# zhizdev/sparsefusion

Measured on AMD Instinct MI355X. Metric: novel views/sec, distillation steps (2 NGP renders fwd+bwd + VAE enc/dec + 51-eval PLMS + LPIPS), 256^2 / 32x32 latents, 2-view synthetic hydrant, higher is better.
Workload: dtype bf16 MFMA operands / f32 accumulate (UNet); f32 (NGP render)

## Files before the change

### include/sparsefusion_hip.h

```cpp
#ifndef SPARSEFUSION_HIP_H
#define SPARSEFUSION_HIP_H

#include <stdint.h>

#ifdef __cplusplus
extern "C" {
#endif

#define SF_OK 0
#define SF_ERR_INVALID 1
#define SF_ERR_LAUNCH 2

const char* sf_last_error(void);
int sf_abi_version(void);
int sf_operand_is_f16(void);


int sf_grid_encode_forward(const float* inputs, const float* embeddings,
                           const int32_t* offsets, float* outputs,
                           uint32_t B, uint32_t D, uint32_t C, uint32_t L,
                           float S, uint32_t H, float* dy_dx,
                           uint32_t gridtype, int align_corners,
                           const int32_t* h_offsets, void* stream);

// ... 116 lines not shown
                         const uint32_t* faces_per_label, const uint32_t* counts3, uint32_t min_faces, double min_fraction,
                         void* workspace, uint64_t workspace_bytes, uint32_t* counts2, void* stream);
int sf_mesh_filter_emit(const float* verts, const int32_t* faces, uint32_t F, uint32_t V, void* workspace,
                        uint64_t workspace_bytes, float* out_verts, int32_t* out_faces, int32_t* vertex_ids, int32_t* face_ids,
                        void* stream);

int sf_ngp_render_forward(const sf_ngp_field* f, const float* rays_o,
                          const float* rays_d, const float* aabb, uint32_t N,
                          uint32_t T, float min_near, const float* lin,
                          const float* u_coarse, const float* u_fine,
                          uint32_t u_fine_row_stride, float bg_color, float* nears,
                          float* fars, float* z_sorted, float* sigma_s,
                          float* rgb_s, float* image, float* depth,
                          float* weights_sum, float* field_cache, float* workspace,
                          uint64_t workspace_bytes, void* stream);

int sf_ngp_render_backward(const sf_ngp_field* f, const sf_ngp_field_grad* g,
                           const float* rays_o, const float* rays_d,
                           const float* aabb, uint32_t N, uint32_t T,
                           const float* nears, const float* fars,
                           const float* z_sorted, const float* sigma_s,
                           const float* rgb_s, float bg_color,
                           const float* grad_image, const float* grad_weights_sum,
                           uint32_t rays_per_row, const float* field_cache,
                           float* workspace, uint64_t workspace_bytes,
                           void* stream);

uint64_t sf_ngp_render_workspace_bytes(uint32_t N, uint32_t T);
uint64_t sf_ngp_render_forward_workspace_bytes(uint32_t N, uint32_t T);

uint64_t sf_ngp_render_cache_bytes(uint32_t N, uint32_t T);

int sf_ngp_field_mfma(int on);

int sf_ngp_field_bwd_pipe(int on);
void sf_ngp_field_bwd_launches(uint64_t* counts);

int sf_ngp_render_shaded_forward(const sf_ngp_field* f, const float* rays_o, const float* rays_d, const float* aabb,
                                 uint32_t N, uint32_t T, float min_near, const float* lin, const float* u_coarse,
                                 const float* u_fine, uint32_t u_fine_row_stride, float bg_color, const float* light_d,
                                 float ambient_ratio, float epsilon, float* nears, float* fars, float* z_sorted,
                                 float* sigma_s, float* rgb_s, float* normal_s, float* rgb_shaded_s, float* xyz_s,
                                 float* image, float* normal_image, float* orient, float* depth, float* weights_sum,
                                 float* workspace, uint64_t workspace_bytes, void* stream);
uint64_t sf_ngp_render_shaded_workspace_bytes(uint32_t N, uint32_t T);

int sf_ngp_render_shaded_forward_train(const sf_ngp_field* f, const float* rays_o, const float* rays_d, const float* aabb,
                                       uint32_t N, uint32_t T, float min_near, const float* lin, const float* u_coarse,
                                       const float* u_fine, uint32_t u_fine_row_stride, float bg_color, const float* light_d,
                                       float ambient_ratio, float epsilon, float* nears, float* fars, float* z_sorted,
                                       float* sigma_s, float* rgb_s, float* normal_s, float* rgb_shaded_s, float* grad_s,
                                       float* w_s, float* image, float* normal_image, float* orient, float* depth,
                                       float* weights_sum, float* workspace, uint64_t workspace_bytes, void* stream);
int sf_ngp_render_shaded_backward(const sf_ngp_field* f, const sf_ngp_field_grad* g, const float* rays_o, const float* rays_d,
                                  const float* aabb, uint32_t N, uint32_t T, const float* nears, const float* fars,
                                  const float* z_sorted, const float* sigma_s, const float* rgb_s, const float* normal_s,
                                  const float* rgb_shaded_s, const float* grad_s, const float* w_s, const float* light_d,
                                  float ambient_ratio, float epsilon, float bg_color, const float* grad_image,
                                  const float* grad_weights_sum, const float* grad_orient, uint32_t rays_per_row,
                                  float* workspace, uint64_t workspace_bytes, void* stream);
uint64_t sf_ngp_render_shaded_backward_workspace_bytes(uint32_t N, uint32_t T);
int sf_ngp_render_offset_backward(const sf_ngp_field* f, const sf_ngp_field_grad* g, const float* rays_o, const float* rays_d,
                                  const float* aabb, uint32_t N, uint32_t T, const float* z_sorted, const float* ds_e, uint32_t e,
                                  float epsilon, uint32_t rays_per_row, float* workspace, uint64_t workspace_bytes, void* stream);

int sf_ngp_render_occ_eval(const sf_ngp_field* f, const float* rays_o, const float* rays_d,
// ... 103 lines not shown
```

### sparsefusion_amd/_lib.py

```python
import ctypes as C
import os

import torch

_HERE = os.path.dirname(os.path.abspath(__file__))
_DEFAULT_LIB = "libsparsefusion_hip_f16.so" if os.environ.get("SF_OPERAND", "bf16").lower() in ("f16", "fp16", "half") else "libsparsefusion_hip.so"
LIB_PATH = os.environ.get("SF_HIP_LIB") or os.path.join(_HERE, _DEFAULT_LIB)

_lib = None

c_f32p = C.c_void_p
c_i32p = C.c_void_p
u32 = C.c_uint32
u64 = C.c_uint64


class SfNgpField(C.Structure):
    _fields_ = [("embeddings", C.c_void_p), ("h_offsets", C.c_void_p), ("L", u32), ("S", C.c_float),
                ("H", u32), ("gridtype", u32),
                ("w0", C.c_void_p), ("b0", C.c_void_p), ("w1", C.c_void_p), ("b1", C.c_void_p),
                ("w2", C.c_void_p), ("b2", C.c_void_p), ("bound", C.c_float)]


class SfNgpFieldGrad(C.Structure):
# ... 51 lines not shown
    "sf_upsample2x_backward": (C.c_int, [c_f32p, c_f32p, u32, u32, u32, C.c_void_p]),
    "sf_render_loss_forward": (C.c_int, [c_f32p, c_f32p, c_f32p, c_f32p, u64, u64, C.c_float, c_f32p, C.c_void_p]),
    "sf_render_loss_backward": (C.c_int, [c_f32p, c_f32p, c_f32p, c_f32p, u64, u64, C.c_float, C.c_float, C.c_float, C.c_float,
                                          C.c_float, c_f32p, c_f32p, c_f32p, C.c_void_p]),
    "sf_fusion_loss_forward": (C.c_int, [c_f32p, c_f32p, c_f32p, c_f32p, u32, u64, u64, c_f32p, C.c_void_p]),
    "sf_fusion_loss_backward": (C.c_int, [c_f32p, c_f32p, c_f32p, c_f32p, u32, u64, u64, C.c_float, C.c_float, C.c_float,
                                          c_f32p, c_f32p, c_f32p, C.c_void_p]),
    "sf_ngp_density": (C.c_int, [C.POINTER(SfNgpField), c_f32p, u32, c_f32p, c_f32p, C.c_void_p]),
    "sf_ngp_density_lattice": (C.c_int, [C.POINTER(SfNgpField), c_f32p, c_f32p, c_f32p, u32, u32, u32, c_f32p, C.c_void_p]),
    "sf_ngp_point_attrs": (C.c_int, [C.POINTER(SfNgpField), c_f32p, u32, C.c_float, c_f32p, c_f32p, c_f32p, c_f32p, C.c_void_p]),
    "sf_ngp_texture_bake": (C.c_int, [C.POINTER(SfNgpField), c_f32p, u32, c_i32p, u32, u32, C.c_void_p, c_f32p, c_f32p, c_i32p,
                                      C.c_void_p]),
    "sf_gaussian3d_workspace_bytes": (u64, [u32, u32, u32]),
    "sf_gaussian3d": (C.c_int, [c_f32p, c_f32p, u32, u32, u32, C.c_float, C.c_float, C.c_void_p, C.c_void_p, u64, C.c_void_p]),
    "sf_mc_workspace_bytes": (u64, [u32, u32, u32]),
    "sf_mc_count": (C.c_int, [c_f32p, u32, u32, u32, C.c_float, C.c_void_p, u64, C.c_void_p, C.c_void_p]),
    "sf_mc_emit": (C.c_int, [c_f32p, u32, u32, u32, C.c_float, C.c_void_p, u64, c_f32p, c_i32p, C.c_void_p]),
    "sf_mesh_components_workspace_bytes": (u64, [u32, u32]),
    "sf_mesh_components": (C.c_int, [c_i32p, u32, u32, c_i32p, c_i32p, C.c_void_p, C.c_void_p, C.c_void_p, u64, C.c_void_p]),
    "sf_mesh_filter_workspace_bytes": (u64, [u32, u32]),
    "sf_mesh_filter_count": (C.c_int, [c_i32p, u32, u32, c_i32p, C.c_void_p, C.c_void_p, u32, C.c_double, C.c_void_p, u64,
                                       C.c_void_p, C.c_void_p]),
    "sf_mesh_filter_emit": (C.c_int, [c_f32p, c_i32p, u32, u32, C.c_void_p, u64, c_f32p, c_i32p, c_i32p, c_i32p, C.c_void_p]),
    "sf_ngp_render_forward": (C.c_int, [C.POINTER(SfNgpField), c_f32p, c_f32p, c_f32p, u32, u32, C.c_float,
                                        c_f32p, c_f32p, c_f32p, u32, C.c_float, c_f32p, c_f32p, c_f32p, c_f32p,
                                        c_f32p, c_f32p, c_f32p, c_f32p, c_f32p, c_f32p, u64, C.c_void_p]),
    "sf_ngp_render_backward": (C.c_int, [C.POINTER(SfNgpField), C.POINTER(SfNgpFieldGrad), c_f32p, c_f32p,
                                         c_f32p, u32, u32, c_f32p, c_f32p, c_f32p, c_f32p, c_f32p,
                                         C.c_float, c_f32p, c_f32p, u32, c_f32p, c_f32p, u64, C.c_void_p]),
    "sf_ngp_render_workspace_bytes": (u64, [u32, u32]),
    "sf_ngp_render_forward_workspace_bytes": (u64, [u32, u32]),
    "sf_ngp_render_cache_bytes": (u64, [u32, u32]),
    "sf_ngp_field_mfma": (C.c_int, [C.c_int]),
    "sf_ngp_field_bwd_pipe": (C.c_int, [C.c_int]),
    "sf_ngp_field_bwd_launches": (None, [C.c_void_p]),
    "sf_ngp_render_shaded_forward": (C.c_int, [C.POINTER(SfNgpField), c_f32p, c_f32p, c_f32p, u32, u32, C.c_float, c_f32p, c_f32p,
                                               c_f32p, u32, C.c_float, c_f32p, C.c_float, C.c_float, c_f32p, c_f32p, c_f32p,
                                               c_f32p, c_f32p, c_f32p, c_f32p, c_f32p, c_f32p, c_f32p, c_f32p, c_f32p, c_f32p,
                                               c_f32p, u64, C.c_void_p]),
    "sf_ngp_render_shaded_workspace_bytes": (u64, [u32, u32]),
    "sf_ngp_render_shaded_forward_train": (C.c_int, [C.POINTER(SfNgpField), c_f32p, c_f32p, c_f32p, u32, u32, C.c_float, c_f32p, c_f32p,
                                                     c_f32p, u32, C.c_float, c_f32p, C.c_float, C.c_float, c_f32p, c_f32p, c_f32p,
                                                     c_f32p, c_f32p, c_f32p, c_f32p, c_f32p, c_f32p, c_f32p, c_f32p, c_f32p, c_f32p,
                                                     c_f32p, c_f32p, u64, C.c_void_p]),
    "sf_ngp_render_shaded_backward": (C.c_int, [C.POINTER(SfNgpField), C.POINTER(SfNgpFieldGrad), c_f32p, c_f32p, c_f32p, u32, u32,
                                                c_f32p, c_f32p, c_f32p, c_f32p, c_f32p, c_f32p, c_f32p, c_f32p, c_f32p, c_f32p,
                                                C.c_float, C.c_float, C.c_float, c_f32p, c_f32p, c_f32p, u32, c_f32p, u64, C.c_void_p]),
    "sf_ngp_render_shaded_backward_workspace_bytes": (u64, [u32, u32]),
    "sf_ngp_render_offset_backward": (C.c_int, [C.POINTER(SfNgpField), C.POINTER(SfNgpFieldGrad), c_f32p, c_f32p, c_f32p, u32, u32, c_f32p,
                                                c_f32p, u32, C.c_float, u32, c_f32p, u64, C.c_void_p]),
    "sf_ngp_render_occ_eval": (C.c_int, [C.POINTER(SfNgpField), c_f32p, c_f32p, c_f32p, c_f32p, C.c_void_p, C.c_float, u32, u32, u32,
                                         c_f32p, C.c_float, u32, c_f32p, c_f32p, c_f32p, C.c_void_p]),
    "sf_ngp_render_occ_eval_shaded": (C.c_int, [C.POINTER(SfNgpField), c_f32p, c_f32p, c_f32p, c_f32p, C.c_void_p, C.c_float, u32, u32,
                                                u32, c_f32p, C.c_float, u32, c_f32p, C.c_float, C.c_float, c_f32p, c_f32p, c_f32p,
                                                c_f32p, C.c_void_p, C.c_void_p]),
    "sf_plan_run": (C.c_int, [C.POINTER(SfOp), u32, C.c_void_p]),
    "sf_conv_igemm_t_launches": (u64, []),
    "sf_gca4_launches": (u64, [C.c_int]),
    "sf_plan_profile": (C.c_int, [C.POINTER(SfOp), u32, C.c_void_p, C.c_void_p]),
    "sf_conv_packed_elems": (u64, [u32, u32, u32, u32]),
    "sf_conv_pack_weights": (C.c_int, [C.c_void_p, u32, u32, u32, u32, u32, C.c_void_p]),
    "sf_plms_update": (C.c_int, [c_f32p, c_f32p, c_f32p, C.c_void_p, u64, c_f32p, c_f32p, C.c_void_p]),
    "sf_plms_combine": (C.c_int, [c_f32p, c_f32p, c_f32p, c_f32p, C.c_void_p, u64, c_f32p, c_f32p, C.c_void_p]),
    "sf_plms_step": (C.c_int, [c_f32p, c_f32p, c_f32p, c_f32p, C.c_void_p, c_f32p, c_f32p, c_f32p, C.c_void_p, u64, c_f32p, c_f32p, c_f32p, u64, C.c_void_p]),
}

# ... 55 lines not shown
```

### sparsefusion_amd/csrc/ngp_field_mfma.h

```cpp
#pragma once
#include "sf_dev.h"
#include "ngp_device.h"

#define FM_PTS 32
#define FM_SF 33
#define FM_SH 65
#define FM_WAVE_FLOATS (FM_PTS * FM_SF + FM_PTS * FM_SH)
#define FM_W2 0
#define FM_B2 (FM_W2 + NGP_OUT * NGP_HID)
#define FM_B0 (FM_B2 + 8)
#define FM_B1 (FM_B0 + NGP_HID)
#define FM_W0 (FM_B1 + NGP_HID)
#define FM_HEAD (FM_W0 + NGP_HID * FM_SF)
#define FM_LDS_FLOATS (FM_HEAD + 4 * FM_WAVE_FLOATS)

#ifndef FM_DEPTH
#define FM_DEPTH 1
#endif

#ifdef SF_HOST_EMU
#define FM_SCHED_FENCE() do { } while (0)
#else
#define FM_SCHED_FENCE() __builtin_amdgcn_sched_barrier(0)
#endif

struct FMArgs {
  const float* table; const float* w0; const float* b0; const float* w1; const float* b1; const float* w2; const float* b2;
  float bound;
  NgpLevels lv;
  const float* rays_o; const float* rays_d; const float* aabb; const float* nears; const float* fars;
  const float* lin; const float* u;
  const float* z_in;
  uint32_t P, T;
  float* z_out;
  float* sigma; float* rgb;
  float* feat_out;
};

SF_DEV void fm_level(const NgpLevels& lv, uint32_t hi, int ll, NgpLevels& m) {
  m.scale[0] = hi ? lv.scale[8 + ll] : lv.scale[ll];
  m.resolution[0] = hi ? lv.resolution[8 + ll] : lv.resolution[ll];
  m.offset[0] = hi ? lv.offset[8 + ll] : lv.offset[ll];
  m.hsize[0] = hi ? lv.hsize[8 + ll] : lv.hsize[ll];
  m.gridtype = lv.gridtype;
}

template <int MODE>
SF_KERNEL(256) void k_ngp_field_mfma(FMArgs a) {
  SF_DYN_LDS(lds_raw);
  float* W = reinterpret_cast<float*>(lds_raw);
  const int tid = threadIdx.x, lane = tid & 63, wave = tid >> 6;
  const int li = lane & 15, kq = lane >> 4;
  float bw1[NGP_HID / 4][4];
  {
    float* S1 = W + FM_HEAD;
    for (int i = tid; i < NGP_HID * NGP_FEAT; i += 256) W[FM_W0 + (i >> 5) * FM_SF + (i & 31)] = a.w0[i];
    for (int i = tid; i < NGP_HID * NGP_HID; i += 256) S1[(i >> 6) * FM_SH + (i & 63)] = a.w1[i];
    for (int i = tid; i < NGP_OUT * NGP_HID; i += 256) W[FM_W2 + i] = a.w2[i];
    if (tid < NGP_HID) { W[FM_B0 + tid] = a.b0[tid]; W[FM_B1 + tid] = a.b1[tid]; }
    if (tid < NGP_OUT) W[FM_B2 + tid] = a.b2[tid];
    sf_sync();
#pragma unroll
    for (int nt = 0; nt < 4; ++nt) {
#pragma unroll
      for (int s = 0; s < NGP_HID / 4; ++s) bw1[s][nt] = S1[(nt * 16 + li) * FM_SH + 4 * s + kq];
    }
    sf_sync();
  }
  float* F = W + FM_HEAD + wave * FM_WAVE_FLOATS;
  float* H = F + FM_PTS * FM_SF;
  float box[6];
#pragma unroll
  for (int i = 0; i < 6; ++i) box[i] = a.aabb[i];

  const int pl = lane & 31, half = lane >> 5;
  const uint32_t n_trips = (a.P + FM_PTS - 1) / FM_PTS;
  for (uint32_t trip = blockIdx.x * 4 + wave; trip < n_trips; trip += gridDim.x * 4) {
    const uint32_t p = trip * FM_PTS + pl;
    const bool live = p < a.P;
    float x01[3] = {0.f, 0.f, 0.f}, blob = 0.0f;
    bool inside = false;
    if (live) {
      const uint32_t n = p / a.T;
      float z;
      if (MODE == 0) {
        z = ngp_coarse_z(a.nears[n], a.fars[n], a.lin[p - n * a.T], a.u ? a.u[p] : -1.0f, a.T);
        if (half == 0) a.z_out[p] = z;
      } else {
        z = a.z_in[p];
      }
      const float o[3] = {a.rays_o[n * 3], a.rays_o[n * 3 + 1], a.rays_o[n * 3 + 2]};
      const float d[3] = {a.rays_d[n * 3], a.rays_d[n * 3 + 1], a.rays_d[n * 3 + 2]};
      float x[3];
      ngp_point(o, d, z, box, x);
      inside = ngp_unit(x, a.bound, x01);
      blob = ngp_blob(x);
    }
    const float xe[3] = {inside ? x01[0] : 0.0f, inside ? x01[1] : 0.0f, inside ? x01[2] : 0.0f};
    uint32_t hi = half;
    SF_USE_FROM_HERE(hi);
    f32x2 fv[FM_DEPTH][8];
    float w[FM_DEPTH][8];
    NgpCell c;
    NgpLevels m;
#pragma unroll
    for (int q = 0; q < FM_DEPTH; ++q) {
      fm_level(a.lv, hi, q, m);
      ngp_cell(m, 0, xe, c);
      const float* tab = a.table + (size_t)m.offset[0] * 2;
#pragma unroll
      for (int i = 0; i < 8; ++i) {
        fv[q][i] = *reinterpret_cast<const f32x2*>(tab + (size_t)c.row[i] * 2);
        w[q][i] = c.w[i];
      }
      FM_SCHED_FENCE();
    }
#pragma unroll
    for (int ll = 0; ll < 8; ++ll) {
      const uint32_t l = hi * 8 + ll;
      const int q = ll % FM_DEPTH;
      const float* tab = a.table;
      if (ll + FM_DEPTH < 8) {
        fm_level(a.lv, hi, ll + FM_DEPTH, m);
        ngp_cell(m, 0, xe, c);
        tab = a.table + (size_t)m.offset[0] * 2;
      }
      FM_SCHED_FENCE();
      float r0 = 0.0f, r1 = 0.0f;
#pragma unroll
      for (int i = 0; i < 8; ++i) {
        r0 = fmaf(w[q][i], fv[q][i][0], r0);
        r1 = fmaf(w[q][i], fv[q][i][1], r1);
      }
      if (!(inside && l < a.lv.L)) r0 = r1 = 0.0f;
      F[pl * FM_SF + 2 * l] = r0;
      F[pl * FM_SF + 2 * l + 1] = r1;
      if (ll + FM_DEPTH < 8) {
#pragma unroll
        for (int i = 0; i < 8; ++i) {
          fv[q][i] = *reinterpret_cast<const f32x2*>(tab + (size_t)c.row[i] * 2);
          w[q][i] = c.w[i];
        }
      }
      FM_SCHED_FENCE();
    }
    if (a.feat_out && live) {
      float* dst = a.feat_out + (size_t)p * NGP_FEAT + half * 16;
#pragma unroll
      for (int j = 0; j < 4; ++j) {
        f32x4 v;
#pragma unroll
        for (int e = 0; e < 4; ++e) v[e] = F[pl * FM_SF + half * 16 + 4 * j + e];
        *reinterpret_cast<f32x4*>(dst + 4 * j) = v;
      }
    }
    sf_wave_sync();

#pragma unroll
    for (int mt = 0; mt < 2; ++mt) {
      f32x4 c[4];
#pragma unroll
      for (int nt = 0; nt < 4; ++nt) {
        const float bv = W[FM_B0 + nt * 16 + li];
        c[nt] = f32x4{bv, bv, bv, bv};
      }
#pragma unroll
      for (int s = 0; s < NGP_FEAT / 4; ++s) {
        const float av = F[(mt * 16 + li) * FM_SF + 4 * s + kq];
#pragma unroll
        for (int nt = 0; nt < 4; ++nt) c[nt] = sf_mfma4(av, W[FM_W0 + (nt * 16 + li) * FM_SF + 4 * s + kq], c[nt]);
      }
#pragma unroll
      for (int nt = 0; nt < 4; ++nt)
#pragma unroll
        for (int r = 0; r < 4; ++r) H[(mt * 16 + 4 * kq + r) * FM_SH + nt * 16 + li] = fmaxf(c[nt][r], 0.0f);
    }
    sf_wave_sync();
#pragma unroll
    for (int mt = 0; mt < 2; ++mt) {
      f32x4 c[4];
#pragma unroll
      for (int nt = 0; nt < 4; ++nt) {
        const float bv = W[FM_B1 + nt * 16 + li];
        c[nt] = f32x4{bv, bv, bv, bv};
      }
#pragma unroll
      for (int s = 0; s < NGP_HID / 4; ++s) {
        const float av = H[(mt * 16 + li) * FM_SH + 4 * s + kq];
#pragma unroll
        for (int nt = 0; nt < 4; ++nt) c[nt] = sf_mfma4(av, bw1[s][nt], c[nt]);
      }
      sf_wave_sync();
#pragma unroll
      for (int nt = 0; nt < 4; ++nt)
#pragma unroll
        for (int r = 0; r < 4; ++r) H[(mt * 16 + 4 * kq + r) * FM_SH + nt * 16 + li] = fmaxf(c[nt][r], 0.0f);
    }
    sf_wave_sync();
    {
      float o0 = W[FM_B2 + 2 * half], o1 = W[FM_B2 + 2 * half + 1];
#pragma unroll 8
      for (int k = 0; k < NGP_HID; ++k) {
        const float hk = H[pl * FM_SH + k];
        o0 = fmaf(W[FM_W2 + (2 * half) * NGP_HID + k], hk, o0);
        o1 = fmaf(W[FM_W2 + (2 * half + 1) * NGP_HID + k], hk, o1);
      }
      if (live) {
        if (half == 0) {
          a.sigma[p] = expf(o0 + blob);
          a.rgb[(size_t)p * 3 + 0] = ngp_sigmoid(o1);
        } else {
          a.rgb[(size_t)p * 3 + 1] = ngp_sigmoid(o0);
          a.rgb[(size_t)p * 3 + 2] = ngp_sigmoid(o1);
        }
      }
    }
    sf_wave_sync();
  }
}
```

### sparsefusion_amd/csrc/ngp_render.hip

```cpp

#include "sf_common.h"
#include "ngp_device.h"
#include "ngp_bwd_plan.h"
#include "ngp_field_lds.h"
#include "ngp_bwd_mfma.h"
#include "ngp_bwd_pipe.h"
#include "ngp_field_mfma.h"
#include "ngp_composite_wave.h"
#include "ngp_scatter_bin.h"
#include "ngp_shade.h"
#include "ngp_shade_bwd.h"
#include <stdlib.h>
#include <atomic>
#include <mutex>

struct GridLevels;
int sf_fill_levels(GridLevels* lv, const int32_t* offsets_dev, const int32_t* h_offsets, uint32_t L, float S,
                   uint32_t H, hipStream_t st);

template <int MODE>
__global__ __launch_bounds__(256) void k_ngp_field(
    FieldPtrs f, NgpLevels lv, const float* __restrict__ rays_o, const float* __restrict__ rays_d,
    const float* __restrict__ aabb, const float* __restrict__ nears, const float* __restrict__ fars,
    const float* __restrict__ lin, const float* __restrict__ u, const float* __restrict__ z_in,
// ... 240 lines not shown
  out->gridtype = f->gridtype;
  return SF_OK;
}

static FieldPtrs field_ptrs(const sf_ngp_field* f) { return sf_ngp_field_ptrs(f); }

extern "C" int sf_ngp_density(const sf_ngp_field* f, const float* xyz, uint32_t P, float* sigma, float* albedo,
                              void* stream) {
  hipStream_t st = (hipStream_t)stream;
  NgpLevels lv;
  if (int rc = sf_ngp_make_levels(f, &lv, st)) return rc;
  if (P == 0) return SF_OK;
  k_ngp_field<2><<<sf_grid_cap(sf_div_up(P, 256)), 256, 0, st>>>(field_ptrs(f), lv, nullptr, nullptr, nullptr, nullptr,
                                                                 nullptr, nullptr, nullptr, nullptr, xyz, P, 1, nullptr,
                                                                 sigma, albedo);
  SF_CHECK_LAUNCH("ngp_density");
  return SF_OK;
}

extern "C" uint64_t sf_ngp_render_workspace_bytes(uint32_t N, uint32_t T) { return ngp_render_workspace_bytes(N, T); }

extern "C" uint64_t sf_ngp_render_forward_workspace_bytes(uint32_t N, uint32_t T) { return ngp_render_forward_workspace_bytes(N, T); }

#ifndef FM_GRID_CAP
#define FM_GRID_CAP 512u
#endif
static std::atomic<int> g_field_mfma{1};
extern "C" int sf_ngp_field_mfma(int on) {
  const int was = g_field_mfma.load(std::memory_order_relaxed);
  if (on >= 0) g_field_mfma.store(on ? 1 : 0, std::memory_order_relaxed);
  return was;
}

static std::atomic<int> g_field_bwd_pipe{SF_FIELD_BWD_PIPE_DEFAULT};
static std::atomic<uint64_t> g_field_bwd_launches[2];
extern "C" int sf_ngp_field_bwd_pipe(int on) {
  const int was = g_field_bwd_pipe.load(std::memory_order_relaxed);
  if (on >= 0) g_field_bwd_pipe.store(on ? 1 : 0, std::memory_order_relaxed);
  return was;
}
extern "C" void sf_ngp_field_bwd_launches(uint64_t* counts) {
  counts[0] = g_field_bwd_launches[0].load(std::memory_order_relaxed);
  counts[1] = g_field_bwd_launches[1].load(std::memory_order_relaxed);
}

extern "C" uint64_t sf_ngp_render_cache_bytes(uint32_t N, uint32_t T) {
  return ((uint64_t)2 * N * T * NGP_FEAT + (uint64_t)N * 2 * T) * sizeof(float);
}

extern "C" int sf_ngp_render_forward(const sf_ngp_field* f, const float* rays_o, const float* rays_d,
                                     const float* aabb, uint32_t N, uint32_t T, float min_near,
                                     const float* lin, const float* u_coarse, const float* u_fine,
                                     uint32_t u_fine_row_stride, float bg_color, float* nears, float* fars,
                                     float* z_sorted, float* sigma_s, float* rgb_s, float* image, float* depth,
                                     float* weights_sum, float* field_cache, float* workspace, uint64_t workspace_bytes,
                                     void* stream) {
  hipStream_t st = (hipStream_t)stream;
  if (N == 0) return SF_OK;
  if (T < 4 || T > 64) SF_FAIL(SF_ERR_INVALID, "ngp_render: T must be in [4,64]");
  if (workspace_bytes < sf_ngp_render_forward_workspace_bytes(N, T)) SF_FAIL(SF_ERR_INVALID, "ngp_render: workspace too small");
  if (!lin || !u_fine) SF_FAIL(SF_ERR_INVALID, "ngp_render: lin and u_fine tables are required");
  NgpLevels lv;
  if (int rc = sf_ngp_make_levels(f, &lv, st)) return rc;
  if (int rc = sf_near_far_from_aabb(rays_o, rays_d, aabb, N, min_near, nears, fars, stream)) return rc;
  const uint64_t NT = (uint64_t)N * T;
  float* z_c = workspace;           float* sig_c = z_c + NT;     float* rgb_c = sig_c + NT;
  float* z_f = rgb_c + 3 * NT;      float* sig_f = z_f + NT;     float* rgb_f = sig_f + NT;
  const FieldPtrs fp = field_ptrs(f);
  const uint32_t P = (uint32_t)NT;
  const uint32_t gridp = sf_grid_cap(sf_div_up(P, 256));
  float* feat_c = field_cache;
  float* feat_f = field_cache ? field_cache + NT * NGP_FEAT : nullptr;
  uint32_t* perm = field_cache ? reinterpret_cast<uint32_t*>(field_cache + 2 * NT * NGP_FEAT) : nullptr;
  const bool mfma = g_field_mfma.load(std::memory_order_relaxed) != 0;
  FMArgs fm{};
  fm.table = fp.table; fm.w0 = fp.w0; fm.b0 = fp.b0; fm.w1 = fp.w1; fm.b1 = fp.b1; fm.w2 = fp.w2; fm.b2 = fp.b2; fm.bound = fp.bound;
  fm.lv = lv; fm.rays_o = rays_o; fm.rays_d = rays_d; fm.aabb = aabb; fm.nears = nears; fm.fars = fars; fm.P = P; fm.T = T;
  const uint32_t gridm = sf_div_up(sf_div_up(P, FM_PTS), 4) < FM_GRID_CAP ? sf_div_up(sf_div_up(P, FM_PTS), 4) : FM_GRID_CAP;
  const size_t ldsm = FM_LDS_FLOATS * sizeof(float);
  if (mfma) {
    fm.lin = lin; fm.u = u_coarse; fm.z_out = z_c; fm.sigma = sig_c; fm.rgb = rgb_c; fm.feat_out = feat_c;
    k_ngp_field_mfma<0><<<gridm, 256, ldsm, st>>>(fm);
  } else {
    k_ngp_field<0><<<gridp, 256, 0, st>>>(fp, lv, rays_o, rays_d, aabb, nears, fars, lin, u_coarse, nullptr, nullptr, P, T,
                                          z_c, sig_c, rgb_c, feat_c);
  }
  SF_CHECK_LAUNCH("ngp_field_coarse");
  const uint32_t gridr = sf_div_up(N, 64);
  k_ngp_sample_fine<<<gridr, 64, 2 * T * 64 * sizeof(float), st>>>(z_c, sig_c, u_fine, u_fine_row_stride, nears, fars,
                                                                  N, T, z_f);
  SF_CHECK_LAUNCH("ngp_sample_fine");
  if (mfma) {
    fm.lin = nullptr; fm.u = nullptr; fm.z_in = z_f; fm.z_out = nullptr; fm.sigma = sig_f; fm.rgb = rgb_f; fm.feat_out = feat_f;
    k_ngp_field_mfma<1><<<gridm, 256, ldsm, st>>>(fm);
  } else {
    k_ngp_field<1><<<gridp, 256, 0, st>>>(fp, lv, rays_o, rays_d, aabb, nears, fars, nullptr, nullptr, z_f, nullptr, P, T,
                                          nullptr, sig_f, rgb_f, feat_f);
  }
  SF_CHECK_LAUNCH("ngp_field_fine");
  k_ngp_composite_wave<<<sf_div_up(N, 4), 256, 4 * 5 * 2 * T * sizeof(float), st>>>(
      CompositeArgs{z_c, sig_c, rgb_c, z_f, sig_f, rgb_f, nears, fars, N, T, bg_color, z_sorted, sigma_s, rgb_s, image, depth,
                    weights_sum, perm});
  SF_CHECK_LAUNCH("ngp_composite");
  return SF_OK;
}

extern "C" uint64_t sf_ngp_render_shaded_workspace_bytes(uint32_t N, uint32_t T) { return sf_ngp_render_forward_workspace_bytes(N, T); }

static int ngp_render_shaded_forward_body(const sf_ngp_field* f, const float* rays_o, const float* rays_d, const float* aabb,
                                          uint32_t N, uint32_t T, float min_near, const float* lin, const float* u_coarse,
                                          const float* u_fine, uint32_t u_fine_row_stride, float bg_color, const float* light_d,
                                          float ambient_ratio, float epsilon, float* nears, float* fars, float* z_sorted,
                                          float* sigma_s, float* rgb_s, float* normal_s, float* rgb_shaded_s, float* xyz_s,
                                          float* grad_s, float* w_s, float* image, float* normal_image, float* orient, float* depth,
                                          float* weights_sum, float* workspace, uint64_t workspace_bytes, void* stream) {
  hipStream_t st = (hipStream_t)stream;
  if (!light_d) SF_FAIL(SF_ERR_INVALID, "ngp_render_shaded: null light_d");
  if (!isfinite(epsilon) || !(epsilon > 0.0f)) SF_FAIL(SF_ERR_INVALID, "ngp_render_shaded: epsilon must be finite and > 0");
  if (!isfinite(ambient_ratio)) SF_FAIL(SF_ERR_INVALID, "ngp_render_shaded: ambient_ratio must be finite");
  if (N == 0) return SF_OK;
  if (T < 4 || T > 64) SF_FAIL(SF_ERR_INVALID, "ngp_render_shaded: T must be in [4,64]");
  if ((uint64_t)N * 2 * T >= (1ull << 32)) SF_FAIL(SF_ERR_INVALID, "ngp_render_shaded: N * 2T must be below 2^32");
  if (workspace_bytes < sf_ngp_render_shaded_workspace_bytes(N, T)) SF_FAIL(SF_ERR_INVALID, "ngp_render_shaded: workspace too small");
  if (!lin || !u_fine) SF_FAIL(SF_ERR_INVALID, "ngp_render_shaded: lin and u_fine tables are required");
  if (!f || !rays_o || !rays_d || !aabb || !nears || !fars || !z_sorted || !sigma_s || !rgb_s || !normal_s || !rgb_shaded_s || !image ||
      !depth || !weights_sum || !workspace)
    SF_FAIL(SF_ERR_INVALID, "ngp_render_shaded: null pointer");
// ... 326 lines not shown
```

### sparsefusion_amd/nerf/renderer.py

```python
import argparse
import ctypes as C
import math
import os

import torch
import torch.nn as nn

from .. import _lib
from .utils import safe_normalize


def get_default_torch_ngp_opt():
    opt = argparse.Namespace()
    opt.cuda_ray = False
    opt.max_steps = 256
    opt.num_steps = 64
    opt.upsample_steps = 64
    opt.update_extra_interval = 16
    opt.max_ray_batch = 4096
    opt.albedo_iters = 1000
    opt.bg_radius = 0
    opt.density_thresh = 10
    opt.fp16 = True
    opt.backbone = 'grid'
# ... 7 lines not shown
    opt.lambda_opacity = 0
    opt.lambda_orient = 1e-2
    opt.lambda_smooth = 0
    opt.shading_backward = False
    return opt


class _FieldHandle:

    def __init__(self, net):
        enc = net.encoder
        lin = net.sigma_net.net
        self.tensors = [enc.embeddings, lin[0].weight, lin[0].bias, lin[1].weight, lin[1].bias, lin[2].weight,
                        lin[2].bias]
        self.host_offsets = enc.host_offsets
        self.L = enc.num_levels
        self.S = float(math.log2(enc.per_level_scale))
        self.H = int(enc.base_resolution)
        self.gridtype = int(enc.gridtype_id)
        self.bound = float(net.bound)

    def struct(self, tensors):
        f = _lib.SfNgpField()
        f.embeddings = tensors[0].data_ptr()
        f.h_offsets = self.host_offsets.ctypes.data
        f.L, f.S, f.H, f.gridtype = self.L, self.S, self.H, self.gridtype
        f.w0, f.b0, f.w1, f.b1, f.w2, f.b2 = (t.data_ptr() for t in tensors[1:])
        f.bound = self.bound
        return f


_FEAT_CACHE = True
_FIELD_MFMA = True
_FIELD_BWD_PIPE = True


def _select_field_kernel(lib):
    lib.sf_ngp_field_mfma(1 if _FIELD_MFMA else 0)


def _select_field_bwd_kernel(lib):
    lib.sf_ngp_field_bwd_pipe(1 if _FIELD_BWD_PIPE else 0)


class _RenderFn(torch.autograd.Function):
    @staticmethod
    def forward(ctx, handle, rays_o, rays_d, aabb, T, min_near, lin, u_coarse, u_fine, u_stride, bg, rays_per_row, grad_mode, *params):
        _lib.require_cuda(rays_o, rays_d, aabb, *params)
        params = [p.detach().contiguous() for p in params]
        N = rays_o.shape[0]
        dev = rays_o.device
        f32 = dict(dtype=torch.float32, device=dev)
        nears, fars = torch.empty(N, **f32), torch.empty(N, **f32)
        z_s, sig_s = torch.empty(N, 2 * T, **f32), torch.empty(N, 2 * T, **f32)
        rgb_s = torch.empty(N, 2 * T, 3, **f32)
        image, depth, ws = torch.empty(N, 3, **f32), torch.empty(N, **f32), torch.empty(N, **f32)
        lib = _lib.lib()
        wbytes = lib.sf_ngp_render_forward_workspace_bytes(N, T)
        work = torch.empty(max(1, wbytes // 4), **f32)
        f = handle.struct(params)
        cache = None
        if _FEAT_CACHE and grad_mode and any(ctx.needs_input_grad[13:]):
            cache = torch.empty(lib.sf_ngp_render_cache_bytes(N, T) // 4, **f32)
        _select_field_kernel(lib)
        rc = lib.sf_ngp_render_forward(C.byref(f), _lib.ptr(rays_o), _lib.ptr(rays_d), _lib.ptr(aabb), N, T,
                                       float(min_near), _lib.ptr(lin), _lib.ptr(u_coarse), _lib.ptr(u_fine),
                                       int(u_stride), float(bg), _lib.ptr(nears), _lib.ptr(fars), _lib.ptr(z_s),
                                       _lib.ptr(sig_s), _lib.ptr(rgb_s), _lib.ptr(image), _lib.ptr(depth), _lib.ptr(ws),
                                       _lib.ptr(cache), _lib.ptr(work), wbytes, _lib.stream_ptr())
        _lib.check(rc, "ngp_render_forward")
        ctx.handle, ctx.T, ctx.bg, ctx.rays_per_row = handle, T, float(bg), int(rays_per_row)
# ... 457 lines not shown
```

Measured before the change: 18.55.

## Software-pipeline NGP field forward: overlap next trip's hash gathers with MLP MFMAs

Restructures the MFMA field forward kernel so each wave encodes the next trip's hash-grid features while running the MLP MFMA steps for the current trip. The encoding is double-buffered in LDS, and scheduler group barriers interleave MFMA and VALU work. The goal is to hide the latency of the gather loads behind matrix work. In exchange it needs more dynamic LDS per block, which may lower occupancy, and it adds a runtime toggle and an attribute call to raise the LDS limit.

```diff
diff --git a/include/sparsefusion_hip.h b/include/sparsefusion_hip.h
--- a/include/sparsefusion_hip.h
+++ b/include/sparsefusion_hip.h
@@ -172,6 +172,8 @@
 uint64_t sf_ngp_render_cache_bytes(uint32_t N, uint32_t T);
 
 int sf_ngp_field_mfma(int on);
+
+int sf_ngp_field_pipe(int on);
 
 int sf_ngp_field_bwd_pipe(int on);
 void sf_ngp_field_bwd_launches(uint64_t* counts);
diff --git a/sparsefusion_amd/_lib.py b/sparsefusion_amd/_lib.py
--- a/sparsefusion_amd/_lib.py
+++ b/sparsefusion_amd/_lib.py
@@ -107,6 +107,7 @@
     "sf_ngp_render_forward_workspace_bytes": (u64, [u32, u32]),
     "sf_ngp_render_cache_bytes": (u64, [u32, u32]),
     "sf_ngp_field_mfma": (C.c_int, [C.c_int]),
+    "sf_ngp_field_pipe": (C.c_int, [C.c_int]),
     "sf_ngp_field_bwd_pipe": (C.c_int, [C.c_int]),
     "sf_ngp_field_bwd_launches": (None, [C.c_void_p]),
     "sf_ngp_render_shaded_forward": (C.c_int, [C.POINTER(SfNgpField), c_f32p, c_f32p, c_f32p, u32, u32, C.c_float, c_f32p, c_f32p,
diff --git a/sparsefusion_amd/csrc/ngp_field_mfma.h b/sparsefusion_amd/csrc/ngp_field_mfma.h
--- a/sparsefusion_amd/csrc/ngp_field_mfma.h
+++ b/sparsefusion_amd/csrc/ngp_field_mfma.h
@@ -6,6 +6,7 @@
 #define FM_SF 33
 #define FM_SH 65
 #define FM_WAVE_FLOATS (FM_PTS * FM_SF + FM_PTS * FM_SH)
+#define FM_PIPE_WAVE_FLOATS (FM_WAVE_FLOATS + FM_PTS * FM_SF)
 #define FM_W2 0
 #define FM_B2 (FM_W2 + NGP_OUT * NGP_HID)
 #define FM_B0 (FM_B2 + 8)
@@ -13,15 +14,22 @@
 #define FM_W0 (FM_B1 + NGP_HID)
 #define FM_HEAD (FM_W0 + NGP_HID * FM_SF)
 #define FM_LDS_FLOATS (FM_HEAD + 4 * FM_WAVE_FLOATS)
-
-#ifndef FM_DEPTH
-#define FM_DEPTH 1
-#endif
+#define FM_PIPE_LDS_FLOATS (FM_HEAD + 4 * FM_PIPE_WAVE_FLOATS)
+#define FM_KSTEPS (2 * NGP_FEAT / 4 + 2 * NGP_HID / 4)
+#define FM_SLOT (FM_KSTEPS / 8)
 
 #ifdef SF_HOST_EMU
 #define FM_SCHED_FENCE() do { } while (0)
+#define FM_SCHED_MIX(n_valu) do { } while (0)
 #else
 #define FM_SCHED_FENCE() __builtin_amdgcn_sched_barrier(0)
+#define FM_SCHED_MIX(n_valu) do { __builtin_amdgcn_sched_group_barrier(0x8, 1, 0); __builtin_amdgcn_sched_group_barrier(0x2, n_valu, 0); } while (0)
+#endif
+#ifndef SF_FIELD_PIPE_DEFAULT
+#define SF_FIELD_PIPE_DEFAULT 1
+#endif
+#ifndef FM_MIX_VALU
+#define FM_MIX_VALU 4
 #endif
 
 struct FMArgs {
@@ -45,7 +53,151 @@
   m.gridtype = lv.gridtype;
 }
 
+struct FMPoint {
+  uint32_t p;
+  bool live, inside;
+  float blob;
+  float xe[3];
+};
+
 template <int MODE>
+SF_DEV void fm_point(const FMArgs& a, const float* box, uint32_t trip, int pl, int half, FMPoint& q) {
+  q.p = trip * FM_PTS + pl;
+  q.live = q.p < a.P;
+  float x01[3] = {0.f, 0.f, 0.f};
+  q.blob = 0.0f;
+  q.inside = false;
+  if (q.live) {
+    const uint32_t p = q.p, n = p / a.T;
+    float z;
+    if (MODE == 0) {
+      z = ngp_coarse_z(a.nears[n], a.fars[n], a.lin[p - n * a.T], a.u ? a.u[p] : -1.0f, a.T);
+      if (half == 0) a.z_out[p] = z;
+    } else {
+      z = a.z_in[p];
+    }
+    const float o[3] = {a.rays_o[n * 3], a.rays_o[n * 3 + 1], a.rays_o[n * 3 + 2]};
+    const float d[3] = {a.rays_d[n * 3], a.rays_d[n * 3 + 1], a.rays_d[n * 3 + 2]};
+    float x[3];
+    ngp_point(o, d, z, box, x);
+    q.inside = ngp_unit(x, a.bound, x01);
+    q.blob = ngp_blob(x);
+  }
+#pragma unroll
+  for (int i = 0; i < 3; ++i) q.xe[i] = q.inside ? x01[i] : 0.0f;
+}
+
+SF_DEV void fm_kstep(int K, f32x4 (&c)[4], const float* F, float* H, const float* W, const float (&bw1)[NGP_HID / 4][4], int li, int kq) {
+  const bool b1 = K < 2 * NGP_FEAT / 4;
+  const int per = b1 ? NGP_FEAT / 4 : NGP_HID / 4, k = b1 ? K : K - 2 * NGP_FEAT / 4;
+  const int mt = k / per, s = k % per;
+  if (s == 0) {
+#pragma unroll
+    for (int nt = 0; nt < 4; ++nt) {
+      const float bv = W[(b1 ? FM_B0 : FM_B1) + nt * 16 + li];
+      c[nt] = f32x4{bv, bv, bv, bv};
+    }
+  }
+  if (b1) {
+    const float av = F[(mt * 16 + li) * FM_SF + 4 * s + kq];
+#pragma unroll
+    for (int nt = 0; nt < 4; ++nt) c[nt] = sf_mfma4(av, W[FM_W0 + (nt * 16 + li) * FM_SF + 4 * s + kq], c[nt]);
+  } else {
+    const float av = H[(mt * 16 + li) * FM_SH + 4 * s + kq];
+#pragma unroll
+    for (int nt = 0; nt < 4; ++nt) c[nt] = sf_mfma4(av, bw1[s][nt], c[nt]);
+  }
+  if (s == per - 1) {
+    if (!b1) sf_wave_sync();
+#pragma unroll
+    for (int nt = 0; nt < 4; ++nt)
+#pragma unroll
+      for (int r = 0; r < 4; ++r) H[(mt * 16 + 4 * kq + r) * FM_SH + nt * 16 + li] = fmaxf(c[nt][r], 0.0f);
+    if (b1 && mt == 1) sf_wave_sync();
+  }
+}
+
+template <bool ENC, bool MLP>
+SF_DEV void fm_trip(const FMArgs& a, const FMPoint& q, float* Fe, const float* F, float* H, const float* W,
+                    const float (&bw1)[NGP_HID / 4][4], int pl, int half, int li, int kq) {
+  uint32_t hi = half;
+  SF_USE_FROM_HERE(hi);
+  f32x2 fv[8];
+  float w[8];
+  f32x4 c[4];
+#pragma unroll
+  for (int r = 0; r <= 8; ++r) {
+    NgpCell cell;
+    const float* tab = a.table;
+    if (ENC && r < 8) {
+      NgpLevels m;
+      fm_level(a.lv, hi, r, m);
+      ngp_cell(m, 0, q.xe, cell);
+      tab = a.table + (size_t)m.offset[0] * 2;
+    }
+    if (MLP && r < 8) {
+#pragma unroll
+      for (int j = 0; j < FM_SLOT; ++j) fm_kstep(r * FM_SLOT + j, c, F, H, W, bw1, li, kq);
+      if (ENC) {
+#pragma unroll
+        for (int j = 0; j < 4 * FM_SLOT; ++j) FM_SCHED_MIX(FM_MIX_VALU);
+      }
+    }
+    FM_SCHED_FENCE();
+    if (ENC && r > 0) {
+      const uint32_t l = hi * 8 + (r - 1);
+      float r0 = 0.0f, r1 = 0.0f;
+#pragma unroll
+      for (int i = 0; i < 8; ++i) {
+        r0 = fmaf(w[i], fv[i][0], r0);
+        r1 = fmaf(w[i], fv[i][1], r1);
+      }
+      if (!(q.inside && l < a.lv.L)) r0 = r1 = 0.0f;
+      Fe[pl * FM_SF + 2 * l] = r0;
+      Fe[pl * FM_SF + 2 * l + 1] = r1;
+    }
+    if (ENC && r < 8) {
+#pragma unroll
+      for (int i = 0; i < 8; ++i) {
+        fv[i] = *reinterpret_cast<const f32x2*>(tab + (size_t)cell.row[i] * 2);
+        w[i] = cell.w[i];
+      }
+    }
+    FM_SCHED_FENCE();
+  }
+  if (ENC && a.feat_out && q.live) {
+    float* dst = a.feat_out + (size_t)q.p * NGP_FEAT + half * 16;
+#pragma unroll
+    for (int j = 0; j < 4; ++j) {
+      f32x4 v;
+#pragma unroll
+      for (int e = 0; e < 4; ++e) v[e] = Fe[pl * FM_SF + half * 16 + 4 * j + e];
+      *reinterpret_cast<f32x4*>(dst + 4 * j) = v;
+    }
+  }
+}
+
+SF_DEV void fm_out(const FMArgs& a, const FMPoint& q, const float* H, const float* W, int pl, int half) {
+  float o0 = W[FM_B2 + 2 * half], o1 = W[FM_B2 + 2 * half + 1];
+#pragma unroll 8
+  for (int k = 0; k < NGP_HID; ++k) {
+    const float hk = H[pl * FM_SH + k];
+    o0 = fmaf(W[FM_W2 + (2 * half) * NGP_HID + k], hk, o0);
+    o1 = fmaf(W[FM_W2 + (2 * half + 1) * NGP_HID + k], hk, o1);
+  }
+  if (q.live) {
+    const uint32_t p = q.p;
+    if (half == 0) {
+      a.sigma[p] = expf(o0 + q.blob);
+      a.rgb[(size_t)p * 3 + 0] = ngp_sigmoid(o1);
+    } else {
+      a.rgb[(size_t)p * 3 + 1] = ngp_sigmoid(o0);
+      a.rgb[(size_t)p * 3 + 2] = ngp_sigmoid(o1);
+    }
+  }
+}
+
+template <int MODE, int PIPE = 0>
 SF_KERNEL(256) void k_ngp_field_mfma(FMArgs a) {
   SF_DYN_LDS(lds_raw);
   float* W = reinterpret_cast<float*>(lds_raw);
@@ -67,154 +219,46 @@
     }
     sf_sync();
   }
-  float* F = W + FM_HEAD + wave * FM_WAVE_FLOATS;
+  float* F = W + FM_HEAD + wave * (PIPE ? FM_PIPE_WAVE_FLOATS : FM_WAVE_FLOATS);
   float* H = F + FM_PTS * FM_SF;
   float box[6];
 #pragma unroll
   for (int i = 0; i < 6; ++i) box[i] = a.aabb[i];
 
   const int pl = lane & 31, half = lane >> 5;
-  const uint32_t n_trips = (a.P + FM_PTS - 1) / FM_PTS;
-  for (uint32_t trip = blockIdx.x * 4 + wave; trip < n_trips; trip += gridDim.x * 4) {
-    const uint32_t p = trip * FM_PTS + pl;
-    const bool live = p < a.P;
-    float x01[3] = {0.f, 0.f, 0.f}, blob = 0.0f;
-    bool inside = false;
-    if (live) {
-      const uint32_t n = p / a.T;
-      float z;
-      if (MODE == 0) {
-        z = ngp_coarse_z(a.nears[n], a.fars[n], a.lin[p - n * a.T], a.u ? a.u[p] : -1.0f, a.T);
-        if (half == 0) a.z_out[p] = z;
-      } else {
-        z = a.z_in[p];
-      }
-      const float o[3] = {a.rays_o[n * 3], a.rays_o[n * 3 + 1], a.rays_o[n * 3 + 2]};
-      const float d[3] = {a.rays_d[n * 3], a.rays_d[n * 3 + 1], a.rays_d[n * 3 + 2]};
-      float x[3];
-      ngp_point(o, d, z, box, x);
-      inside = ngp_unit(x, a.bound, x01);
-      blob = ngp_blob(x);
-    }
-    const float xe[3] = {inside ? x01[0] : 0.0f, inside ? x01[1] : 0.0f, inside ? x01[2] : 0.0f};
-    uint32_t hi = half;
-    SF_USE_FROM_HERE(hi);
-    f32x2 fv[FM_DEPTH][8];
-    float w[FM_DEPTH][8];
-    NgpCell c;
-    NgpLevels m;
-#pragma unroll
-    for (int q = 0; q < FM_DEPTH; ++q) {
-      fm_level(a.lv, hi, q, m);
-      ngp_cell(m, 0, xe, c);
-      const float* tab = a.table + (size_t)m.offset[0] * 2;
-#pragma unroll
-      for (int i = 0; i < 8; ++i) {
-        fv[q][i] = *reinterpret_cast<const f32x2*>(tab + (size_t)c.row[i] * 2);
-        w[q][i] = c.w[i];
-      }
-      FM_SCHED_FENCE();
-    }
-#pragma unroll
-    for (int ll = 0; ll < 8; ++ll) {
-      const uint32_t l = hi * 8 + ll;
-      const int q = ll % FM_DEPTH;
-      const float* tab = a.table;
-      if (ll + FM_DEPTH < 8) {
-        fm_level(a.lv, hi, ll + FM_DEPTH, m);
-        ngp_cell(m, 0, xe, c);
-        tab = a.table + (size_t)m.offset[0] * 2;
-      }
-      FM_SCHED_FENCE();
-      float r0 = 0.0f, r1 = 0.0f;
-#pragma unroll
-      for (int i = 0; i < 8; ++i) {
-        r0 = fmaf(w[q][i], fv[q][i][0], r0);
-        r1 = fmaf(w[q][i], fv[q][i][1], r1);
-      }
-      if (!(inside && l < a.lv.L)) r0 = r1 = 0.0f;
-      F[pl * FM_SF + 2 * l] = r0;
-      F[pl * FM_SF + 2 * l + 1] = r1;
-      if (ll + FM_DEPTH < 8) {
-#pragma unroll
-        for (int i = 0; i < 8; ++i) {
-          fv[q][i] = *reinterpret_cast<const f32x2*>(tab + (size_t)c.row[i] * 2);
-          w[q][i] = c.w[i];
-        }
-      }
-      FM_SCHED_FENCE();
-    }
-    if (a.feat_out && live) {
-      float* dst = a.feat_out + (size_t)p * NGP_FEAT + half * 16;
-#pragma unroll
-      for (int j = 0; j < 4; ++j) {
-        f32x4 v;
-#pragma unroll
-        for (int e = 0; e < 4; ++e) v[e] = F[pl * FM_SF + half * 16 + 4 * j + e];
-        *reinterpret_cast<f32x4*>(dst + 4 * j) = v;
-      }
-    }
-    sf_wave_sync();
-
-#pragma unroll
-    for (int mt = 0; mt < 2; ++mt) {
-      f32x4 c[4];
-#pragma unroll
-      for (int nt = 0; nt < 4; ++nt) {
-        const float bv = W[FM_B0 + nt * 16 + li];
-        c[nt] = f32x4{bv, bv, bv, bv};
-      }
-#pragma unroll
-      for (int s = 0; s < NGP_FEAT / 4; ++s) {
-        const float av = F[(mt * 16 + li) * FM_SF + 4 * s + kq];
-#pragma unroll
-        for (int nt = 0; nt < 4; ++nt) c[nt] = sf_mfma4(av, W[FM_W0 + (nt * 16 + li) * FM_SF + 4 * s + kq], c[nt]);
-      }
-#pragma unroll
-      for (int nt = 0; nt < 4; ++nt)
-#pragma unroll
-        for (int r = 0; r < 4; ++r) H[(mt * 16 + 4 * kq + r) * FM_SH + nt * 16 + li] = fmaxf(c[nt][r], 0.0f);
-    }
-    sf_wave_sync();
-#pragma unroll
-    for (int mt = 0; mt < 2; ++mt) {
-      f32x4 c[4];
-#pragma unroll
-      for (int nt = 0; nt < 4; ++nt) {
-        const float bv = W[FM_B1 + nt * 16 + li];
-        c[nt] = f32x4{bv, bv, bv, bv};
-      }
-#pragma unroll
-      for (int s = 0; s < NGP_HID / 4; ++s) {
-        const float av = H[(mt * 16 + li) * FM_SH + 4 * s + kq];
-#pragma unroll
-        for (int nt = 0; nt < 4; ++nt) c[nt] = sf_mfma4(av, bw1[s][nt], c[nt]);
-      }
+  const uint32_t n_trips = (a.P + FM_PTS - 1) / FM_PTS, stride = gridDim.x * 4;
+  if (!PIPE) {
+    for (uint32_t trip = blockIdx.x * 4 + wave; trip < n_trips; trip += stride) {
+      FMPoint q;
+      fm_point<MODE>(a, box, trip, pl, half, q);
+      fm_trip<true, false>(a, q, F, F, H, W, bw1, pl, half, li, kq);
       sf_wave_sync();
-#pragma unroll
-      for (int nt = 0; nt < 4; ++nt)
-#pragma unroll
-        for (int r = 0; r < 4; ++r) H[(mt * 16 + 4 * kq + r) * FM_SH + nt * 16 + li] = fmaxf(c[nt][r], 0.0f);
-    }
-    sf_wave_sync();
-    {
-      float o0 = W[FM_B2 + 2 * half], o1 = W[FM_B2 + 2 * half + 1];
-#pragma unroll 8
-      for (int k = 0; k < NGP_HID; ++k) {
-        const float hk = H[pl * FM_SH + k];
-        o0 = fmaf(W[FM_W2 + (2 * half) * NGP_HID + k], hk, o0);
-        o1 = fmaf(W[FM_W2 + (2 * half + 1) * NGP_HID + k], hk, o1);
-      }
-      if (live) {
-        if (half == 0) {
-          a.sigma[p] = expf(o0 + blob);
-          a.rgb[(size_t)p * 3 + 0] = ngp_sigmoid(o1);
-        } else {
-          a.rgb[(size_t)p * 3 + 1] = ngp_sigmoid(o0);
-          a.rgb[(size_t)p * 3 + 2] = ngp_sigmoid(o1);
-        }
-      }
-    }
-    sf_wave_sync();
-  }
-}
+      fm_trip<false, true>(a, q, F, F, H, W, bw1, pl, half, li, kq);
+      sf_wave_sync();
+      fm_out(a, q, H, W, pl, half);
+      sf_wave_sync();
+    }
+  } else {
+    float* Fn = H + FM_PTS * FM_SH;
+    const uint32_t t0 = blockIdx.x * 4 + (uint32_t)sf_uniform(wave);
+    if (t0 < n_trips) {
+      FMPoint q, qn = {}, q2 = {};
+      fm_point<MODE>(a, box, t0, pl, half, q);
+      fm_trip<true, false>(a, q, F, F, H, W, bw1, pl, half, li, kq);
+      uint32_t next = t0 + stride;
+      if (next < n_trips) fm_point<MODE>(a, box, next, pl, half, qn);
+      for (;;) {
+        sf_wave_sync();
+        if (next < n_trips) fm_trip<true, true>(a, qn, Fn, F, H, W, bw1, pl, half, li, kq);
+        else fm_trip<false, true>(a, q, F, F, H, W, bw1, pl, half, li, kq);
+        sf_wave_sync();
+        if (next + stride < n_trips) fm_point<MODE>(a, box, next + stride, pl, half, q2);
+        fm_out(a, q, H, W, pl, half);
+        sf_wave_sync();
+        if (next >= n_trips) break;
+        q = qn; qn = q2; next += stride;
+        float* t = F; F = Fn; Fn = t;
+      }
+    }
+  }
+}
diff --git a/sparsefusion_amd/csrc/ngp_render.hip b/sparsefusion_amd/csrc/ngp_render.hip
--- a/sparsefusion_amd/csrc/ngp_render.hip
+++ b/sparsefusion_amd/csrc/ngp_render.hip
@@ -296,6 +296,25 @@
   return was;
 }
 
+static std::atomic<int> g_field_pipe{SF_FIELD_PIPE_DEFAULT};
+extern "C" int sf_ngp_field_pipe(int on) {
+  const int was = g_field_pipe.load(std::memory_order_relaxed);
+  if (on >= 0) g_field_pipe.store(on ? 1 : 0, std::memory_order_relaxed);
+  return was;
+}
+static std::atomic<bool> g_field_pipe_lds[32];
+static int ngp_field_pipe_raise_lds() {
+  int dev_id = 0;
+  if (hipGetDevice(&dev_id) != hipSuccess) SF_FAIL(SF_ERR_LAUNCH, "hipGetDevice failed");
+  if (dev_id >= 0 && dev_id < 32 && g_field_pipe_lds[dev_id].load(std::memory_order_acquire)) return SF_OK;
+  const int bytes = (int)(FM_PIPE_LDS_FLOATS * sizeof(float));
+  if (hipFuncSetAttribute(reinterpret_cast<const void*>(&k_ngp_field_mfma<0, 1>), hipFuncAttributeMaxDynamicSharedMemorySize, bytes) != hipSuccess ||
+      hipFuncSetAttribute(reinterpret_cast<const void*>(&k_ngp_field_mfma<1, 1>), hipFuncAttributeMaxDynamicSharedMemorySize, bytes) != hipSuccess)
+    SF_FAIL(SF_ERR_LAUNCH, "ngp_render: cannot raise the dynamic LDS limit of the pipelined field forward");
+  if (dev_id >= 0 && dev_id < 32) g_field_pipe_lds[dev_id].store(true, std::memory_order_release);
+  return SF_OK;
+}
+
 static std::atomic<int> g_field_bwd_pipe{SF_FIELD_BWD_PIPE_DEFAULT};
 static std::atomic<uint64_t> g_field_bwd_launches[2];
 extern "C" int sf_ngp_field_bwd_pipe(int on) {
@@ -341,10 +360,14 @@
   fm.table = fp.table; fm.w0 = fp.w0; fm.b0 = fp.b0; fm.w1 = fp.w1; fm.b1 = fp.b1; fm.w2 = fp.w2; fm.b2 = fp.b2; fm.bound = fp.bound;
   fm.lv = lv; fm.rays_o = rays_o; fm.rays_d = rays_d; fm.aabb = aabb; fm.nears = nears; fm.fars = fars; fm.P = P; fm.T = T;
   const uint32_t gridm = sf_div_up(sf_div_up(P, FM_PTS), 4) < FM_GRID_CAP ? sf_div_up(sf_div_up(P, FM_PTS), 4) : FM_GRID_CAP;
-  const size_t ldsm = FM_LDS_FLOATS * sizeof(float);
+  const bool pipe = mfma && g_field_pipe.load(std::memory_order_relaxed) != 0;
+  const size_t ldsm = (pipe ? FM_PIPE_LDS_FLOATS : FM_LDS_FLOATS) * sizeof(float);
+  if (pipe)
+    if (int rc = ngp_field_pipe_raise_lds()) return rc;
   if (mfma) {
     fm.lin = lin; fm.u = u_coarse; fm.z_out = z_c; fm.sigma = sig_c; fm.rgb = rgb_c; fm.feat_out = feat_c;
-    k_ngp_field_mfma<0><<<gridm, 256, ldsm, st>>>(fm);
+    if (pipe) k_ngp_field_mfma<0, 1><<<gridm, 256, ldsm, st>>>(fm);
+    else k_ngp_field_mfma<0, 0><<<gridm, 256, ldsm, st>>>(fm);
   } else {
     k_ngp_field<0><<<gridp, 256, 0, st>>>(fp, lv, rays_o, rays_d, aabb, nears, fars, lin, u_coarse, nullptr, nullptr, P, T,
                                           z_c, sig_c, rgb_c, feat_c);
@@ -356,7 +379,8 @@
   SF_CHECK_LAUNCH("ngp_sample_fine");
   if (mfma) {
     fm.lin = nullptr; fm.u = nullptr; fm.z_in = z_f; fm.z_out = nullptr; fm.sigma = sig_f; fm.rgb = rgb_f; fm.feat_out = feat_f;
-    k_ngp_field_mfma<1><<<gridm, 256, ldsm, st>>>(fm);
+    if (pipe) k_ngp_field_mfma<1, 1><<<gridm, 256, ldsm, st>>>(fm);
+    else k_ngp_field_mfma<1, 0><<<gridm, 256, ldsm, st>>>(fm);
   } else {
     k_ngp_field<1><<<gridp, 256, 0, st>>>(fp, lv, rays_o, rays_d, aabb, nears, fars, nullptr, nullptr, z_f, nullptr, P, T,
                                           nullptr, sig_f, rgb_f, feat_f);
diff --git a/sparsefusion_amd/nerf/renderer.py b/sparsefusion_amd/nerf/renderer.py
--- a/sparsefusion_amd/nerf/renderer.py
+++ b/sparsefusion_amd/nerf/renderer.py
@@ -63,11 +63,13 @@
 
 _FEAT_CACHE = True
 _FIELD_MFMA = True
+_FIELD_PIPE = True
 _FIELD_BWD_PIPE = True
 
 
 def _select_field_kernel(lib):
     lib.sf_ngp_field_mfma(1 if _FIELD_MFMA else 0)
+    lib.sf_ngp_field_pipe(1 if _FIELD_PIPE else 0)
 
 
 def _select_field_bwd_kernel(lib):
```

Result: no change. 18.52 (-0.2%).
